# AY-Liu/Image-Editing-Framework

Measured on AMD Instinct MI355X. Metric: denoising steps/sec (SD1.5 512x512 P2P edit step, UNet batch 4), higher is better.
Workload: dtype f16x3; 1 GPU; sd15 UNet (859.5M params) P2P AttentionRefine edit step, 2 prompts x CFG = batch 4, 64x64 latents (512x512 px), 50-step DDIM, guidance 7.5, cross 0.8 / self 0.4, per-step null-text unconditional embeddings (P2P_NTI, edit_real.py); one independent edit per GPU; precision mode f16x3: fp32 storage; every contraction on split operands: hi + lo fp16 halves of each fp32 element, Ah Bh + Al Bh + Ah Bl =

## Files before the change

image-editing-framework_amd/csrc/split_x3.hip:

```cpp
#include "ief_common.h"
#include "ief_params.h"

#include "x3_common.h"

__global__ __launch_bounds__(256) void x3_split_weights_kernel(const float* __restrict__ w, half_t* __restrict__ planes, long long n4,
                                                               float s) {
    for (long long i = (long long)blockIdx.x * 256 + threadIdx.x; i < n4; i += (long long)gridDim.x * 256) {
        half4 h, l;
        split4(((const f32x4*)w)[i], s, h, l);
        ((half4*)planes)[i] = h;
        ((half4*)planes)[n4 + i] = l;
    }
}
extern "C" int ief_x3_split_weights(const float* w, void* planes, long long n, float scale, void* stream) {
    if (!w || !planes) return IEF_EINVAL;
    if (n <= 0 || (n & 3) || !(scale > 0.f)) return IEF_ESHAPE;
    long long grid = (n / 4 + 255) / 256;
    if (grid > 16384) grid = 16384;
    hipLaunchKernelGGL(x3_split_weights_kernel, dim3((unsigned)grid), dim3(256), 0, (hipStream_t)stream, w, (half_t*)planes, n / 4, scale);
    IEF_LAUNCH_CHECK();
    return IEF_OK;
}

template <int WM, int WN, int TM, int TN, int KIND, bool TRANSB, bool BPRE>
__global__ __launch_bounds__(64 * WM * WN, (2 * 2 * 16 * (WM * TM + WN * TN) * YLD * 2 > 80 * 1024) ? (WM * WN) / 4 : (WM * WN) / 2)
void igemm_x3_kernel(const IefGemmF32Params p) {
    constexpr bool CONV = KIND >= X3_CONV;
    constexpr bool HASFAST = KIND == X3_LIN || KIND == X3_CONV;
    constexpr int NTH = 64 * WM * WN;
    constexpr int BM = 16 * WM * TM, BN = 16 * WN * TN;
    constexpr int ROWS = BM + BN;
    constexpr int NA = (BM * 8 + NTH - 1) / NTH;
    constexpr int NBC = BPRE ? 2 * BN * 4 : BN * 8;
    constexpr int NB = (NBC + NTH - 1) / NTH;
    constexpr bool A_EXACT = (BM * 8) % NTH == 0, B_EXACT = NBC % NTH == 0;
    static_assert(!(BPRE && TRANSB), "pre-split planes are [N][K]");
    constexpr unsigned OOB = 0xFFFFFFF0u;
    constexpr unsigned OOBF = 0x80000000u;
    __shared__ __attribute__((aligned(16))) half_t smem_y[2 * 2 * ROWS * YLD];
    const int tid = threadIdx.x, lane = tid & 63, wid = tid >> 6;
    const int wm = wid / WN, wn = wid - wm * WN;
    const int lr = lane & 15, lg = lane >> 4;
    const int ntn = (p.N + BN - 1) / BN;
    const int ntiles = ((p.M + BM - 1) / BM) * ntn;
    const int bid = xcd_remap(blockIdx.x, ntiles);
    const int ntm = (p.M + BM - 1) / BM;
    const int grp = bid / (X3_GROUP_M * ntn), within = bid - grp * (X3_GROUP_M * ntn);
    const int gsz = min(X3_GROUP_M, ntm - grp * X3_GROUP_M);
    const int tn = within / gsz, tm = grp * X3_GROUP_M + (within - tn * gsz);
    const int m0 = tm * BM, n0 = tn * BN;
    const float* A = p.A;
    const float* W = p.W;
    float* Out = p.Out;
    if (p.heads > 0) {
        const int b = blockIdx.z / p.heads, h = blockIdx.z - b * p.heads;
        const int ba = p.a_src ? p.a_src[b] : b, bw = p.w_src ? p.w_src[b] : b;
        A += (long long)ba * p.sAb + (long long)h * p.sAh;
        W += (long long)bw * p.sWb + (long long)h * p.sWh;
        Out += (long long)b * p.sOb + (long long)h * p.sOh;
    }
    const int M = p.M, N = p.N, K = p.K;
    const float sa = p.sa, sb = p.sb;
    const int kc4 = (tid & 7) * 4;
    const int rq = tid >> 3;
    const int r0 = (rq & ~3) | ((rq & 1) << 1) | ((rq >> 1) & 1);
    constexpr int RSTEP = NTH / 8;
    RowCoordY rc[NA];
    unsigned pixo1[NA], pixo2[NA], tmask[NA];
    if (CONV) {
#pragma unroll
        for (int i = 0; i < NA; ++i) {
            const int m = m0 + r0 + RSTEP * i;
            rc[i].ok = m < M && (A_EXACT || r0 + RSTEP * i < BM);
            const int mm = rc[i].ok ? m : 0;
            const int hw = p.Ho * p.Wo;
            rc[i].b = mm / hw;
            const int rem = mm - rc[i].b * hw;
            rc[i].oy = rem / p.Wo;
            rc[i].ox = rem - rc[i].oy * p.Wo;
            if (KIND == X3_CONV) {
                const int pl = p.pad_hi_only ? 0 : 1;
                const unsigned pix = (unsigned)((rc[i].b * p.H + rc[i].oy * p.stride) * p.Wd + rc[i].ox * p.stride);
                pixo1[i] = pix * (unsigned)p.C1 * 4u; pixo2[i] = pix * (unsigned)p.C2 * 4u;
                unsigned mk = 0;
#pragma unroll
                for (int t = 0; t < 9; ++t) {
                    const int iy = rc[i].oy * p.stride + t / 3 - pl, ix = rc[i].ox * p.stride + t % 3 - pl;
                    mk |= (rc[i].ok && (unsigned)iy < (unsigned)p.H && (unsigned)ix < (unsigned)p.Wd) ? (1u << t) : 0u;
                }
                tmask[i] = mk;
            }
        }
    }
    const int Ct = p.C1 + p.C2, K9 = 9 * Ct;
    const int pad_lo = p.pad_hi_only ? 0 : 1;
    const int Hs = p.ups ? (p.H >> 1) : p.H, Ws = p.ups ? (p.Wd >> 1) : p.Wd;

    const int nk_all = (K + YBK - 1) / YBK;
    int kt0 = 0, nk = nk_all;
    if (p.splits > 1) {
        const int per = (nk_all + p.splits - 1) / p.splits;
        kt0 = blockIdx.y * per;
        nk = min(per, nk_all - kt0);
        if (nk < 0) nk = 0;
    }
    const int kend = min(K, (kt0 + nk) * YBK);

    const rsrc_t rA = make_rsrc(A, p.bytesA), rW = make_rsrc(BPRE ? (const void*)p.Wp : (const void*)W, p.bytesW);
    const rsrc_t rA2 = make_rsrc(p.A2, p.bytesA2), rE1 = make_rsrc(p.E1, p.bytesE1), rE2 = make_rsrc(p.E2, p.bytesE2);
    unsigned aoff[NA], boff[NB];
    bool aval[NA], bval[NB];
    int bq8[NB];
    int bldsoff[NB];
#pragma unroll
    for (int i = 0; i < NA; ++i) {
        const int ml = r0 + RSTEP * i, m = m0 + ml;
        aval[i] = (m < M) & (A_EXACT || ml < BM);
        aoff[i] = (unsigned)((m * p.lda + kc4) * 4);
    }
#pragma unroll
    for (int i = 0; i < NB; ++i) {
        bq8[i] = 0;
        if (BPRE) {
            const int c = tid + NTH * i;
            const int plane = c >= BN * 4 ? 1 : 0, cc = c - plane * BN * 4;
            const int rr = cc >> 2, q = cc & 3;
            const int nl = (rr & ~3) | ((rr & 1) << 1) | ((rr >> 1) & 1), n = n0 + nl;
            bval[i] = (c < NBC) & (n < N);
            bq8[i] = q * 8;
            boff[i] = (unsigned)(((long long)plane * N * K + (long long)n * K + q * 8) * 2);
            bldsoff[i] = plane * BN * YLD + nl * YLD + q * 8;
        } else if (!TRANSB) {
            const int nl = r0 + RSTEP * i, n = n0 + nl;
            bval[i] = (n < N) & (B_EXACT || nl < BN);
            boff[i] = (unsigned)((n * p.ldw + kc4) * 4);
            bldsoff[i] = nl * YLD + kc4;
        } else {
            const int c = tid + NTH * i;
            const int nl = (c >> 5) * 4, n = n0 + nl;
            bval[i] = (n < N) & (B_EXACT || nl < BN);
            boff[i] = (unsigned)(((c & 31) * p.ldw + n) * 4);
            bldsoff[i] = nl * YLD + (c & 31);
        }
    }

    auto load_tile = [&](int k0, f32x4 (&ra)[NA], f32x4 (&rb)[NB]) {
        const int kk = k0 + kc4;
        if (KIND == X3_CONV || KIND == X3_CONV_UPS) {
            int tap = 9, ch = k0 - K9;
            if (k0 < K9) { tap = k0 / Ct; ch = k0 - tap * Ct; }
            rsrc_t rs = rA;
            int cs = p.C1, chs = ch, ky = 0, kx = 0;
            const bool tapm = tap < 9;
            bool second = false;
            if (tapm) {
                ky = (tap * 11) >> 5; kx = tap - 3 * ky;
                if (ch >= p.C1) { rs = rA2; cs = p.C2; chs = ch - p.C1; second = true; }
            } else if (ch < p.CE1) { rs = rE1; cs = p.CE1; }
            else { rs = rE2; cs = p.CE2; chs = ch - p.CE1; }
            const int kin = k0 < kend ? 1 : 0;
            if (KIND == X3_CONV) {
                const int uni = tapm ? (((ky - pad_lo) * p.Wd + (kx - pad_lo)) * cs + chs) * 4 : chs * 4;
                const unsigned bit = tapm ? (1u << tap) : 0u;
                const unsigned cs4 = (unsigned)cs * 4u;
#pragma unroll
                for (int i = 0; i < NA; ++i) {
                    const unsigned base = tapm ? (second ? pixo2[i] : pixo1[i]) : (unsigned)(m0 + r0 + RSTEP * i) * cs4;
                    const bool ok = tapm ? (tmask[i] & bit) != 0 : rc[i].ok != 0;
                    ra[i] = bload(rs, (ok & (kin != 0)) ? base + (unsigned)uni + (unsigned)(kc4 * 4) : OOB);
                }
            } else {
                const int dy = tapm ? ky - pad_lo : 0, dx = tapm ? kx - pad_lo : 0;
                const unsigned Hc = tapm ? p.H : p.Ho, Wc = tapm ? p.Wd : p.Wo;
                const int sh = tapm ? 1 : 0;
                const int hs = tapm ? Hs : p.Ho, ws = tapm ? Ws : p.Wo;
                const int cb = chs + kc4;
#pragma unroll
                for (int i = 0; i < NA; ++i) {
                    const int iy = rc[i].oy + dy, ix = rc[i].ox + dx;
                    const int ok = rc[i].ok & kin & ((unsigned)iy < Hc ? 1 : 0) & ((unsigned)ix < Wc ? 1 : 0);
                    const unsigned off = (unsigned)((((rc[i].b * hs + (iy >> sh)) * ws + (ix >> sh)) * cs + cb) * 4);
                    ra[i] = bload(rs, ok ? off : OOB);
                }
            }
        } else if (KIND == X3_CONV_SLOW) {
            const float* src = nullptr;
            int cs = 0, chs = 0, ky = 0, kx = 0, mode = 0;
            if (kk < K9 && kk < kend) {
                const int tap = kk / Ct, ch = kk - tap * Ct;
                ky = tap / 3; kx = tap - 3 * ky;
                if (ch < p.C1) { src = p.A; cs = p.C1; chs = ch; } else { src = p.A2; cs = p.C2; chs = ch - p.C1; }
                mode = 1;
            } else if (kk < kend) {
                const int ch2 = kk - K9;
                if (ch2 < p.CE1) { src = p.E1; cs = p.CE1; chs = ch2; } else { src = p.E2; cs = p.CE2; chs = ch2 - p.CE1; }
                mode = 2;
            }
#pragma unroll
            for (int i = 0; i < NA; ++i) {
                f32x4 v = {0.f, 0.f, 0.f, 0.f};
                if (rc[i].ok && mode == 1) {
                    int iy = rc[i].oy * p.stride + ky - pad_lo, ix = rc[i].ox * p.stride + kx - pad_lo;
                    if ((unsigned)iy < (unsigned)p.H && (unsigned)ix < (unsigned)p.Wd) {
                        if (p.ups) { iy >>= 1; ix >>= 1; }
                        v = *(const f32x4*)(src + (((long long)rc[i].b * Hs + iy) * Ws + ix) * cs + chs);
                    }
                } else if (rc[i].ok && mode == 2) {
                    v = *(const f32x4*)(src + (((long long)rc[i].b * p.Ho + rc[i].oy) * p.Wo + rc[i].ox) * cs + chs);
                }
                ra[i] = v;
            }
        } else if (KIND == X3_LIN) {
#pragma unroll
            for (int i = 0; i < NA; ++i) ra[i] = bload(rA, (aval[i] & (kk < kend)) ? aoff[i] + (unsigned)(k0 * 4) : OOB);
        } else {
#pragma unroll
            for (int i = 0; i < NA; ++i) {
                const int m = m0 + r0 + RSTEP * i;
                f32x4 v = {0.f, 0.f, 0.f, 0.f};
                if (m < M && kk < kend && (A_EXACT || r0 + RSTEP * i < BM)) {
                    const float* ap = A + (long long)m * p.lda + kk;
#pragma unroll
                    for (int j = 0; j < 4; ++j) if (kk + j < K) v[j] = ap[j];
                }
                ra[i] = v;
            }
        }
        if (BPRE) {
#pragma unroll
            for (int i = 0; i < NB; ++i) rb[i] = bload(rW, (bval[i] & (k0 + bq8[i] < kend)) ? boff[i] + (unsigned)(k0 * 2) : OOB);
        } else if (!TRANSB) {
#pragma unroll
            for (int i = 0; i < NB; ++i) rb[i] = bload(rW, (bval[i] & (kk < kend)) ? boff[i] + (unsigned)(k0 * 4) : OOB);
        } else {
#pragma unroll
            for (int i = 0; i < NB; ++i) {
                const int kr = k0 + ((tid + NTH * i) & 31);
                rb[i] = bload(rW, (bval[i] & (kr < kend)) ? boff[i] + (unsigned)(k0 * p.ldw * 4) : OOB);
            }
        }
    };

    unsigned afast[NA], bfast[NB];
    rsrc_t f_rs = rA;
    int f_tap = 0, f_ch = 0, f_left = 0, f_uni = 0;
#pragma unroll
    for (int i = 0; i < NA; ++i) afast[i] = aval[i] ? aoff[i] : OOBF;
#pragma unroll
    for (int i = 0; i < NB; ++i) bfast[i] = bval[i] ? boff[i] : OOBF;
    auto seg_setup = [&]() {
        int cs, chs, src_c;
        const bool tapm = f_tap < 9;
        bool second = false;
        if (tapm) {
            if (f_ch >= p.C1) { f_rs = rA2; cs = p.C2; chs = f_ch - p.C1; second = true; src_c = p.C2; }
            else { f_rs = rA; cs = p.C1; chs = f_ch; src_c = p.C1; }
        } else if (f_ch < p.CE1) { f_rs = rE1; cs = p.CE1; chs = f_ch; src_c = p.CE1; }
        else { f_rs = rE2; cs = p.CE2; chs = f_ch - p.CE1; src_c = p.CE2; }
        f_left = (src_c - chs) / YBK;
        f_uni = chs * 4;
        const int ky = (f_tap * 11) >> 5, kx = f_tap - 3 * ky;
        const int tapoff = tapm ? ((ky - pad_lo) * p.Wd + (kx - pad_lo)) * cs * 4 : 0;
        const unsigned bit = tapm ? (1u << f_tap) : 0u;
#pragma unroll
        for (int i = 0; i < NA; ++i) {
            const unsigned base = tapm ? (second ? pixo2[i] : pixo1[i]) + (unsigned)tapoff
                                       : (unsigned)(m0 + r0 + RSTEP * i) * (unsigned)cs * 4u;
            const bool ok = tapm ? (tmask[i] & bit) != 0 : rc[i].ok != 0;
            afast[i] = ok ? base + (unsigned)(kc4 * 4) : OOBF;
        }
    };
    auto load_fast = [&](int k0, f32x4 (&ra)[NA], f32x4 (&rb)[NB]) {
        if (KIND == X3_CONV) {
#pragma unroll
            for (int i = 0; i < NA; ++i) ra[i] = bload(f_rs, afast[i] + (unsigned)f_uni);
            f_uni += YBK * 4;
            f_ch += YBK;
            if (--f_left == 0) {
                if (f_tap < 9 && f_ch >= Ct) { f_ch = 0; ++f_tap; }
                seg_setup();
            }
        } else {
#pragma unroll
            for (int i = 0; i < NA; ++i) ra[i] = bload(rA, afast[i] + (unsigned)(k0 * 4));
        }
        const unsigned kb = BPRE ? (unsigned)(k0 * 2) : TRANSB ? (unsigned)(k0 * p.ldw * 4) : (unsigned)(k0 * 4);
#pragma unroll
        for (int i = 0; i < NB; ++i) rb[i] = bload(rW, bfast[i] + kb);
    };

    auto store_chunk = [&](int buf, int idx, const f32x4 (&ra)[NA], const f32x4 (&rb)[NB]) {
        half_t* ah = smem_y + buf * (2 * ROWS * YLD);
        half_t* al = ah + BM * YLD;
        half_t* bh = al + BM * YLD;
        half_t* bl = bh + BN * YLD;
        if (idx < NA) {
            const int i = idx;
            if (!A_EXACT && r0 + RSTEP * i >= BM) return;
            half4 h, l;
            split4(ra[i], sa, h, l);
            const int off = (r0 + RSTEP * i) * YLD + kc4;
            *(half4*)(ah + off) = h;
            *(half4*)(al + off) = l;
        } else if (BPRE) {
            const int i = idx - NA;
            if (!B_EXACT && tid + NTH * i >= NBC) return;
            *(f32x4*)(bh + bldsoff[i]) = rb[i];
        } else if (!TRANSB) {
            const int i = idx - NA;
            if (!B_EXACT && r0 + RSTEP * i >= BN) return;
            half4 h, l;
            split4(rb[i], sb, h, l);
            *(half4*)(bh + bldsoff[i]) = h;
            *(half4*)(bl + bldsoff[i]) = l;
        } else {
            const int i = idx - NA;
            if (!B_EXACT && ((tid + NTH * i) >> 5) * 4 >= BN) return;
            half4 h, l;
            split4(rb[i], sb, h, l);
#pragma unroll
            for (int j = 0; j < 4; ++j) {
                bh[bldsoff[i] + j * YLD] = h[j];
                bl[bldsoff[i] + j * YLD] = l[j];
            }
        }
    };
    auto store_tile = [&](int buf, const f32x4 (&ra)[NA], const f32x4 (&rb)[NB]) {
#pragma unroll
        for (int c = 0; c < NA + NB; ++c) store_chunk(buf, c, ra, rb);
    };

    f32x4 acc[TN][TM];
#pragma unroll
    for (int b = 0; b < TN; ++b)
#pragma unroll
        for (int a = 0; a < TM; ++a) acc[b][a] = f32x4{0.f, 0.f, 0.f, 0.f};

    auto mma_tile = [&](int buf, const f32x4 (&ra)[NA], const f32x4 (&rb)[NB]) {
        const half_t* ah = smem_y + buf * (2 * ROWS * YLD) + (wm * TM * 16 + lr) * YLD + 8 * lg;
        const half_t* al = ah + BM * YLD;
        const half_t* bh = smem_y + buf * (2 * ROWS * YLD) + 2 * BM * YLD + (wn * TN * 16 + lr) * YLD + 8 * lg;
        const half_t* bl = bh + BN * YLD;
        half8_t fah[TM], fal[TM];
#pragma unroll
        for (int a = 0; a < TM; ++a) {
            fah[a] = *(const half8_t*)(ah + a * 16 * YLD);
            fal[a] = *(const half8_t*)(al + a * 16 * YLD);
        }
#pragma unroll
        for (int b = 0; b < TN; ++b) {
            const half8_t fbh = *(const half8_t*)(bh + b * 16 * YLD);
            const half8_t fbl = *(const half8_t*)(bl + b * 16 * YLD);
#pragma unroll
            for (int a = 0; a < TM; ++a) {
                acc[b][a] = __builtin_amdgcn_mfma_f32_16x16x32_f16(fbl, fah[a], acc[b][a], 0, 0, 0);
                acc[b][a] = __builtin_amdgcn_mfma_f32_16x16x32_f16(fbh, fal[a], acc[b][a], 0, 0, 0);
                acc[b][a] = __builtin_amdgcn_mfma_f32_16x16x32_f16(fbh, fah[a], acc[b][a], 0, 0, 0);
            }
        }
        store_tile(buf ^ 1, ra, rb);
    };

    f32x4 ra0[NA], rb0[NB], ra1[NA], rb1[NB];
    load_tile(kt0 * YBK, ra0, rb0);
    load_tile((kt0 + 1) * YBK, ra1, rb1);
    store_tile(0, ra0, rb0);
    __syncthreads();
    int kt = 0;
    if (HASFAST && p.fast_ok) {
        const int nfast = kend / YBK - kt0;
        if (KIND == X3_CONV && nfast > 3) {
            const int k0 = (kt0 + 2) * YBK;
            if (k0 < K9) { f_tap = k0 / Ct; f_ch = k0 - f_tap * Ct; } else { f_tap = 9; f_ch = k0 - K9; }
            seg_setup();
        }
        for (; kt + 3 < nfast; kt += 2) {
            load_fast((kt0 + kt + 2) * YBK, ra0, rb0);
            mma_tile(0, ra1, rb1);
            __syncthreads();
            load_fast((kt0 + kt + 3) * YBK, ra1, rb1);
            mma_tile(1, ra0, rb0);
            __syncthreads();
        }
    }
    for (; kt < nk; kt += 2) {
        load_tile((kt0 + kt + 2) * YBK, ra0, rb0);
        mma_tile(0, ra1, rb1);
        __syncthreads();
        load_tile((kt0 + kt + 3) * YBK, ra1, rb1);
        mma_tile(1, ra0, rb0);
        __syncthreads();
    }
    const float inv = 1.0f / (sa * sb);
    const bool vec = p.vec_out != 0;
    if (p.splits > 1) {
        float* slab = p.ws + (long long)blockIdx.y * M * N;
#pragma unroll
        for (int a = 0; a < TM; ++a) {
            const int m = m0 + (wm * TM + a) * 16 + lr;
            if (m >= M) continue;
#pragma unroll
            for (int b = 0; b < TN; ++b) {
                const int n = n0 + (wn * TN + b) * 16 + 4 * lg;
                if (n >= N) continue;
                const f32x4 v = acc[b][a] * inv;
                if ((N & 3) == 0) *(f32x4*)(slab + (long long)m * N + n) = v;
                else {
#pragma unroll
                    for (int j = 0; j < 4; ++j) if (n + j < N) slab[(long long)m * N + n + j] = v[j];
                }
            }
        }
        return;
    }
    if (p.geglu) {
#pragma unroll
        for (int a = 0; a < TM; ++a) {
            const int m = m0 + (wm * TM + a) * 16 + lr;
#pragma unroll
            for (int b = 0; b < TN; ++b) {
                const int n = n0 + (wn * TN + b) * 16 + 4 * lg;
                f32x4 v = acc[b][a] * inv;
                if (p.bias && n < N) v += *(const f32x4*)(p.bias + n);
                f32x4 g;
#pragma unroll
                for (int j = 0; j < 4; ++j) g[j] = __shfl_xor(v[j], 32);
                if (lg < 2 && m < M && n < N) {
                    f32x4 o;
#pragma unroll
                    for (int j = 0; j < 4; ++j) o[j] = v[j] * gelu_f(g[j]) * p.out_scale;
                    *(f32x4*)(Out + (long long)m * p.ldo + (n0 + (wn * TN + b) * 16) / 2 + 4 * lg) = o;
                }
            }
        }
        return;
    }
    const float* R = p.residual;
#pragma unroll
    for (int a = 0; a < TM; ++a) {
        const int m = m0 + (wm * TM + a) * 16 + lr;
        if (m >= M) continue;
        const float* rv = p.rowvec ? p.rowvec + (long long)(m / p.rows_per_batch) * N : nullptr;
#pragma unroll
        for (int b = 0; b < TN; ++b) {
            const int n = n0 + (wn * TN + b) * 16 + 4 * lg;
            if (n >= N) continue;
            f32x4 v = acc[b][a] * inv;
            if (vec) {
                if (p.bias) v += *(const f32x4*)(p.bias + n);
                if (rv) v += *(const f32x4*)(rv + n);
                if (R) v += *(const f32x4*)(R + (long long)m * p.ldr + n);
                *(f32x4*)(Out + (long long)m * p.ldo + n) = v * p.out_scale;
            } else {
#pragma unroll
                for (int j = 0; j < 4; ++j) {
                    if (n + j >= N) break;
                    float s = v[j];
                    if (p.bias) s += p.bias[n + j];
                    if (rv) s += rv[n + j];
                    if (R) s += R[(long long)m * p.ldr + n + j];
                    Out[(long long)m * p.ldo + n + j] = s * p.out_scale;
                }
            }
        }
    }
}

static int g_x3_wide = 1, g_flash_ks2 = 1;
extern "C" void ief_gemm_x3_set_variant(int v) { g_x3_wide = v & 1; g_flash_ks2 = (v & 2) ? 0 : 1; }
static bool x3_wide_ok(int conv, int N, int K) { return g_x3_wide && N % 160 == 0 && (conv || N <= 1280 || K >= 1280); }
extern "C" int ief_gemm_x3_bn_k(int conv, int N, int K) { return x3_wide_ok(conv, N, K) ? 160 : (N % 80 == 0) ? 80 : 64; }
extern "C" int ief_gemm_x3_bn(int N) { return (N % 80 == 0) ? 80 : 64; }
extern "C" int ief_gemm_x3_bm(int M, int N) {
    (void)M; (void)N;
    return 128;
}

template <int WM, int WN, int TM, int TN, int KIND, bool TRANSB, bool BPRE>
static int launch_igemm_x3(const IefGemmF32Params& p, hipStream_t st) {
    constexpr int BM = 16 * WM * TM, BN = 16 * WN * TN;
    const int tiles = ((p.M + BM - 1) / BM) * ((p.N + BN - 1) / BN);
    const int z = p.heads > 0 ? p.batch * p.heads : 1;
    const int splits = p.splits > 1 ? p.splits : 1;
    hipLaunchKernelGGL((igemm_x3_kernel<WM, WN, TM, TN, KIND, TRANSB, BPRE>), dim3(tiles, splits, z), dim3(64 * WM * WN), 0, st, p);
    IEF_LAUNCH_CHECK();
    return IEF_OK;
}

int ief_gemm_x3_dispatch(const IefGemmF32Params& pin, hipStream_t st) {
    IefGemmF32Params p = pin;
    const bool al = ((p.N & 3) == 0) && ((p.ldo & 3) == 0) && (((uintptr_t)p.Out & 15) == 0) &&
                    (!p.bias || ((uintptr_t)p.bias & 15) == 0) && (!p.rowvec || ((uintptr_t)p.rowvec & 15) == 0) &&
                    (!p.residual || (((uintptr_t)p.residual & 15) == 0 && (p.ldr & 3) == 0)) &&
                    (p.heads == 0 || (((p.sOb | p.sOh) & 3) == 0));
    p.vec_out = al ? 1 : 0;
    if (p.geglu && (p.conv || p.transb || p.heads > 0 || p.splits > 1 || (p.N & 15) || p.residual || p.rowvec || !al ||
                    (((uintptr_t)p.Out | (uintptr_t)(p.bias ? p.bias : p.Out)) & 15) || (p.ldo & 3)))
        return IEF_EINVAL;
    const bool bpre = p.Wp != nullptr;
    if (bpre && (p.transb || p.heads > 0 || (p.K & 7) || ((uintptr_t)p.Wp & 15) || (!p.conv && p.ldw != p.K))) return IEF_EINVAL;
    const unsigned long long lim = 0xFFFFFFF0ull;
    unsigned long long bA, bW, bA2 = 0, bE1 = 0, bE2 = 0;
    if (p.conv) {
        const unsigned long long px = (unsigned long long)p.batch_images * (p.ups ? (p.H >> 1) * (p.Wd >> 1) : p.H * p.Wd);
        bA = px * p.C1 * 4; bA2 = px * p.C2 * 4;
        bE1 = (unsigned long long)p.M * p.CE1 * 4; bE2 = (unsigned long long)p.M * p.CE2 * 4;
        p.al32 = ((p.C1 | p.C2 | p.CE1 | p.CE2) & 31) == 0 ? 1 : 0;
    } else {
        bA = ((unsigned long long)(p.M - 1) * p.lda + p.K) * 4;
        p.al32 = 0;
    }
    bW = bpre ? 4ull * p.N * p.K
              : p.transb ? ((unsigned long long)(p.K - 1) * p.ldw + p.N) * 4 : ((unsigned long long)(p.N - 1) * p.ldw + p.K) * 4;
    if (bA >= lim || bW >= lim || bA2 >= lim || bE1 >= lim || bE2 >= lim) return IEF_ESHAPE;
    p.bytesA = (unsigned)bA; p.bytesW = (unsigned)bW; p.bytesA2 = (unsigned)bA2; p.bytesE1 = (unsigned)bE1; p.bytesE2 = (unsigned)bE2;
    const unsigned long long half = 0x40000000ull;
    const unsigned long long kspan = p.transb ? 4ull * p.K * p.ldw : 4ull * p.K;
    p.fast_ok = (bA < half && bW < half && bA2 < half && bE1 < half && bE2 < half && kspan < half) ? 1 : 0;
    if (x3_wide_ok(p.conv, p.N, p.K) && bpre && !p.a_scalar && (!p.conv || (p.al32 && !p.ups)))
        return p.conv ? launch_igemm_x3<4, 2, 2, 5, X3_CONV, false, true>(p, st) : launch_igemm_x3<4, 2, 2, 5, X3_LIN, false, true>(p, st);
    const bool n80 = p.N % 80 == 0;
#define X3_GO(KIND_, TRANSB_, BPRE_) (n80 ? launch_igemm_x3<4, 1, 2, 5, KIND_, TRANSB_, BPRE_>(p, st) \
                                          : launch_igemm_x3<2, 2, 4, 2, KIND_, TRANSB_, BPRE_>(p, st))
    if (p.conv) {
        if (!p.al32) return bpre ? X3_GO(X3_CONV_SLOW, false, true) : X3_GO(X3_CONV_SLOW, false, false);
        if (p.ups) return bpre ? X3_GO(X3_CONV_UPS, false, true) : X3_GO(X3_CONV_UPS, false, false);
        return bpre ? X3_GO(X3_CONV, false, true) : X3_GO(X3_CONV, false, false);
    }
    if (p.transb) return p.a_scalar ? X3_GO(X3_LIN_SLOW, true, false) : X3_GO(X3_LIN, true, false);
    if (p.a_scalar) return bpre ? X3_GO(X3_LIN_SLOW, false, true) : X3_GO(X3_LIN_SLOW, false, false);
    return bpre ? X3_GO(X3_LIN, false, true) : X3_GO(X3_LIN, false, false);
#undef X3_GO
}

template <int D, int KS>
__global__ __launch_bounds__(256, (D > 80) ? 1 : 2) void attn_flash_x3_kernel(const IefAttnF32Params p) {
    constexpr int DG = (D + 15) / 16;
    constexpr int DT = (D + 31) / 32;
    constexpr int KLD = DG * 16 + 8;
    constexpr int KT = 32 * KS;
    constexpr int VRS = D <= 32 ? 32 : (D <= 96 ? 96 : 160);
    static_assert(VRS >= 32 * DT, "V row covers the padded head dim");
    constexpr float SQ = 1.f, SK = 1.f, SV = 1.f, SP = 16384.f;
    __shared__ __attribute__((aligned(16))) half_t smem_f[2 * KT * KLD + 2 * KT * VRS];
    half_t* Kh = smem_f;
    half_t* Kl = Kh + KT * KLD;
    half_t* Vh = Kl + KT * KLD;
    half_t* Vl = Vh + KT * VRS;
    const int tid = threadIdx.x, lane = tid & 63, wid = tid >> 6;
    const int li = lane & 31, lh = lane >> 5;
    const int nqb = gridDim.x;
    const int lid = xcd_remap(blockIdx.x + nqb * blockIdx.y, nqb * gridDim.y);
    const int bh = lid / nqb, qb = lid - bh * nqb, b = bh / p.heads, h = bh - b * p.heads;
    const int bq = p.q_src ? p.q_src[b] : b, bk = p.k_src ? p.k_src[b] : b, bv = p.v_src ? p.v_src[b] : b;
    const float* Q = p.Q + (long long)bq * p.sQb + (long long)h * D;
    const float* Kp = p.K + (long long)bk * p.sKb + (long long)h * D;
    const float* Vp = p.V + (long long)bv * p.sVb + (long long)h * D;
    float* O = p.Out ? p.Out + (long long)b * p.sOb + (long long)h * D : nullptr;
    half_t* OP = p.OutP ? p.OutP + (long long)b * p.sOPb + (long long)h * D : nullptr;
    const int q0 = qb * 128 + wid * 32;
    const int qi = q0 + li;
    for (int c = tid; c < (int)(sizeof(smem_f) / 16); c += 256) ((f32x4*)smem_f)[c] = f32x4{0.f, 0.f, 0.f, 0.f};
    half8_t qh[DG], ql[DG];
#pragma unroll
    for (int g = 0; g < DG; ++g) {
#pragma unroll
        for (int c2 = 0; c2 < 2; ++c2) {
            const int d0 = g * 16 + 8 * lh + 4 * c2;
            f32x4 v = {0.f, 0.f, 0.f, 0.f};
            if (qi < p.N && d0 < D) v = *(const f32x4*)(Q + (long long)qi * p.ldq + d0);
            half4 hh, ll;
            split4(v, SQ, hh, ll);
#pragma unroll
            for (int j = 0; j < 4; ++j) { qh[g][4 * c2 + j] = hh[j]; ql[g][4 * c2 + j] = ll[j]; }
        }
    }
    f32x16 o[DT];
#pragma unroll
    for (int t = 0; t < DT; ++t)
#pragma unroll
        for (int r = 0; r < 16; ++r) o[t][r] = 0.f;
    float m_run = -INFINITY, l_run = 0.f;
    const float sc2 = p.scale * 1.44269504088896341f / (SQ * SK);
    constexpr int KCH = KT * (D / 4);
    constexpr int NLD = (KCH + 255) / 256;
    const rsrc_t rK = make_rsrc(Kp, (unsigned)(((long long)(p.L - 1) * p.ldk + D) * 4));
    const rsrc_t rV = make_rsrc(Vp, (unsigned)(((long long)(p.L - 1) * p.ldv + D) * 4));
    f32x4 rk[NLD], rv[NLD];
    auto load_kv = [&](int k0) {
#pragma unroll
        for (int i = 0; i < NLD; ++i) {
            const int c = tid + 256 * i;
            const int row = c / (D / 4), ch = c - row * (D / 4);
            const bool ok = (c < KCH) & (k0 + row < p.L);
            rk[i] = bload(rK, ok ? (unsigned)(((k0 + row) * p.ldk + ch * 4) * 4) : 0xFFFFFFF0u);
            rv[i] = bload(rV, ok ? (unsigned)(((k0 + row) * p.ldv + ch * 4) * 4) : 0xFFFFFFF0u);
        }
    };
    auto store_kv = [&]() {
#pragma unroll
        for (int i = 0; i < NLD; ++i) {
            const int c = tid + 256 * i;
            if (c < KCH) {
                const int row = c / (D / 4), ch = c - row * (D / 4);
                half4 hh, ll;
                split4(rk[i], SK, hh, ll);
                *(half4*)(Kh + row * KLD + ch * 4) = hh;
                *(half4*)(Kl + row * KLD + ch * 4) = ll;
                split4(rv[i], SV, hh, ll);
                *(half4*)(Vh + row * VRS + ch * 4) = hh;
                *(half4*)(Vl + row * VRS + ch * 4) = ll;
            }
        }
    };
    const int L16 = lane & 15;
    const int v_lane = (4 * lh + (L16 >> 2)) * VRS + 16 * ((lane >> 4) & 1) + 4 * (L16 & 3);
    const int nt = (p.L + KT - 1) / KT;
    load_kv(0);
    for (int t = 0; t < nt; ++t) {
        __syncthreads();
        store_kv();
        __syncthreads();
        load_kv((t + 1) * KT);
        f32x16 sacc[KS];
#pragma unroll
        for (int u = 0; u < KS; ++u) {
#pragma unroll
            for (int r = 0; r < 16; ++r) sacc[u][r] = 0.f;
#pragma unroll
            for (int g = 0; g < DG; ++g) {
                const half8_t kh = *(const half8_t*)(Kh + (u * 32 + li) * KLD + g * 16 + 8 * lh);
                const half8_t kl = *(const half8_t*)(Kl + (u * 32 + li) * KLD + g * 16 + 8 * lh);
                sacc[u] = __builtin_amdgcn_mfma_f32_32x32x16_f16(kl, qh[g], sacc[u], 0, 0, 0);
                sacc[u] = __builtin_amdgcn_mfma_f32_32x32x16_f16(kh, ql[g], sacc[u], 0, 0, 0);
                sacc[u] = __builtin_amdgcn_mfma_f32_32x32x16_f16(kh, qh[g], sacc[u], 0, 0, 0);
            }
        }
#pragma unroll
        for (int u = 0; u < KS; ++u) {
            if (t * KT + (u + 1) * 32 > p.L) {
#pragma unroll
                for (int r = 0; r < 16; ++r) {
                    const int key = t * KT + u * 32 + (r & 3) + 8 * (r >> 2) + 4 * lh;
                    if (key >= p.L) sacc[u][r] = -INFINITY;
                }
            }
        }
        float mxa = -INFINITY, mxb = -INFINITY;
#pragma unroll
        for (int r = 0; r < 8; ++r) {
            if (KS == 2) {
                mxa = __builtin_fmaxf(__builtin_fmaxf(mxa, sacc[0][r]), sacc[KS - 1][r]);
                mxb = __builtin_fmaxf(__builtin_fmaxf(mxb, sacc[0][8 + r]), sacc[KS - 1][8 + r]);
            } else {
                mxa = __builtin_fmaxf(mxa, sacc[0][r]);
                mxb = __builtin_fmaxf(mxb, sacc[0][8 + r]);
            }
        }
        float mx = fmaxf(mxa, mxb) * sc2;
        mx = fmaxf(mx, __shfl_xor(mx, 32));
        const float m_new = fmaxf(m_run, mx);
        const float alpha = __builtin_amdgcn_exp2f(m_run - m_new);
        float ls = 0.f;
#pragma unroll
        for (int u = 0; u < KS; ++u)
#pragma unroll
            for (int r = 0; r < 16; ++r) { sacc[u][r] = __builtin_amdgcn_exp2f(__builtin_fmaf(sacc[u][r], sc2, -m_new)); ls += sacc[u][r]; }
        l_run = l_run * alpha + ls;
        if (__builtin_amdgcn_ballot_w64(m_new != m_run) != 0) {
#pragma unroll
            for (int tt = 0; tt < DT; ++tt)
#pragma unroll
                for (int r = 0; r < 16; ++r) o[tt][r] *= alpha;
        }
        m_run = m_new;
#pragma unroll
        for (int u = 0; u < KS; ++u) {
#pragma unroll
            for (int s = 0; s < 2; ++s) {
                half8_t ph, pl;
#pragma unroll
                for (int c2 = 0; c2 < 2; ++c2) {
                    const f32x4 v = {sacc[u][8 * s + 4 * c2], sacc[u][8 * s + 4 * c2 + 1], sacc[u][8 * s + 4 * c2 + 2], sacc[u][8 * s + 4 * c2 + 3]};
                    half4 hh, ll;
                    split4(v, SP, hh, ll);
#pragma unroll
                    for (int j = 0; j < 4; ++j) { ph[4 * c2 + j] = hh[j]; pl[4 * c2 + j] = ll[j]; }
                }
#pragma unroll
                for (int tt = 0; tt < DT; ++tt) {
                    const int vo = v_lane + (u * 32 + 16 * s) * VRS + 32 * tt;
                    const half4 a0 = x3_lds_tr_read(Vh + vo), a1 = x3_lds_tr_read(Vh + vo + 8 * VRS);
                    const half4 b0 = x3_lds_tr_read(Vl + vo), b1 = x3_lds_tr_read(Vl + vo + 8 * VRS);
                    half8_t vh, vl;
#pragma unroll
                    for (int j = 0; j < 4; ++j) { vh[j] = a0[j]; vh[4 + j] = a1[j]; vl[j] = b0[j]; vl[4 + j] = b1[j]; }
                    o[tt] = __builtin_amdgcn_mfma_f32_32x32x16_f16(vl, ph, o[tt], 0, 0, 0);
                    o[tt] = __builtin_amdgcn_mfma_f32_32x32x16_f16(vh, pl, o[tt], 0, 0, 0);
                    o[tt] = __builtin_amdgcn_mfma_f32_32x32x16_f16(vh, ph, o[tt], 0, 0, 0);
                }
            }
        }
    }
    const float l_tot = l_run + __shfl_xor(l_run, 32);
    const float inv = 1.0f / (l_tot * SV * SP);
    if (p.lse && qi < p.N && lh == 0) p.lse[((long long)b * p.heads + h) * p.N + qi] = m_run + __log2f(l_tot);
    if (qi < p.N) {
#pragma unroll
        for (int tt = 0; tt < DT; ++tt)
#pragma unroll
            for (int g = 0; g < 4; ++g) {
                const int d = tt * 32 + 8 * g + 4 * lh;
                if (d < D) {
                    const f32x4 v = {o[tt][4 * g] * inv, o[tt][4 * g + 1] * inv, o[tt][4 * g + 2] * inv, o[tt][4 * g + 3] * inv};
                    if (O) *(f32x4*)(O + (long long)qi * p.ldo + d) = v;
                    if (OP) {
                        half4 hh, ll;
                        split4(v, 1.0f, hh, ll);
                        half_t* op = OP + (long long)qi * p.ldp + d;
                        *(half4*)op = hh;
                        *(half4*)(op + p.planeO) = ll;
                    }
                }
            }
    }
}


#ifndef X3P_FLASH_BATCH_READS
#define X3P_FLASH_BATCH_READS 1
#endif
template <int D, int KS, int NWV>
__global__ __launch_bounds__(64 * NWV, D <= 40 ? 4 : 2) void attn_flash_x3p_kernel(const IefAttnF32Params p) {
    constexpr int DG = (D + 15) / 16, DT = (D + 31) / 32;
    constexpr int KT = 32 * KS;
    constexpr int CPR = D / 8;
    constexpr int PL = KT * D;
    constexpr int NP = PL * 2 / 1024;
    static_assert((PL * 2) % 1024 == 0, "a plane of a tile is a whole number of LDS-DMA pieces");
    constexpr bool SWZ = D == 64;
    constexpr float LOGSP = 10.f, THR = 5.f;
    constexpr bool BATCH_READS = X3P_FLASH_BATCH_READS != 0;
    __shared__ __attribute__((aligned(1024))) half_t smem_p[2 * 4 * PL];
    const int tid = threadIdx.x, lane = tid & 63;
    const int wid = __builtin_amdgcn_readfirstlane(tid >> 6);
    const int li = lane & 31, lh = lane >> 5;
    const int nqb = gridDim.x;
    const int lid = xcd_remap(blockIdx.x + nqb * blockIdx.y, nqb * gridDim.y);
    const int bh = lid / nqb, qb = lid - bh * nqb, b = bh / p.heads, h = bh - b * p.heads;
    const int bq = p.q_src ? p.q_src[b] : b, bk = p.k_src ? p.k_src[b] : b, bv = p.v_src ? p.v_src[b] : b;
    const half_t* Qh = p.Qp + (long long)bq * p.sQb + (long long)h * D;
    const char* srcs[4];
#pragma unroll
    for (int pl = 0; pl < 4; ++pl)
        srcs[pl] = (const char*)(pl < 2 ? p.Kp + (long long)bk * p.sKb + (pl & 1) * p.planeK
                                        : p.Vp + (long long)bv * p.sVb + (pl & 1) * p.planeV) + (long long)h * D * 2;
    const char* zp = (const char*)p.zeros;
    float* O = p.Out ? p.Out + (long long)b * p.sOb + (long long)h * D : nullptr;
    half_t* OP = p.OutP ? p.OutP + (long long)b * p.sOPb + (long long)h * D : nullptr;
    const int q0 = qb * (32 * NWV) + wid * 32;
    const int qi = q0 + li;
    half8_t qh[DG], ql[DG];
#pragma unroll
    for (int g = 0; g < DG; ++g) {
        const int d0 = g * 16 + 8 * lh;
        if (qi < p.N && d0 < D) {
            qh[g] = *(const half8_t*)(Qh + (long long)qi * p.ldq + d0);
            ql[g] = *(const half8_t*)(Qh + p.planeQ + (long long)qi * p.ldq + d0);
        } else {
#pragma unroll
            for (int j = 0; j < 8; ++j) { qh[g][j] = 0; ql[g][j] = 0; }
        }
    }
    constexpr int NPW = (4 * NP + NWV - 1) / NWV;
    int s_row[NPW];
    unsigned s_off[NPW];
#pragma unroll
    for (int i = 0; i < NPW; ++i) {
        const int q = wid + NWV * i, j = q % NP;
        const int c = 64 * j + lane;
        s_row[i] = c / CPR;
        const int ch = c - s_row[i] * CPR;
        s_off[i] = (unsigned)((SWZ ? (ch ^ (s_row[i] & 7)) : ch) * 16);
    }
    auto issue = [&](int t, int buf) {
#pragma unroll
        for (int i = 0; i < NPW; ++i) {
            const int q = wid + NWV * i;
            if (q < 4 * NP) {
                const int pl = q / NP, j = q - pl * NP;
                const int row = t * KT + s_row[i];
                const int ldr = pl < 2 ? p.ldk : p.ldv;
                const char* g = row < p.L ? srcs[pl] + (long long)row * ldr * 2 + s_off[i] : zp;
                x3_glds16(g, smem_p + buf * (4 * PL) + pl * PL + j * 512);
            }
        }
    };
    int koff[DG];
#pragma unroll
    for (int g = 0; g < DG; ++g) {
        const int chunk = (g * 16 + 8 * lh < D) ? 2 * g + lh : 0;
        koff[g] = li * D + (SWZ ? ((chunk ^ (li & 7)) << 3) : (chunk << 3));
    }
    const int L16 = lane & 15;
    const int vrow = 4 * lh + (L16 >> 2);
    int voff[DT];
#pragma unroll
    for (int tt = 0; tt < DT; ++tt) {
        int col = 32 * tt + 16 * ((lane >> 4) & 1) + 4 * (L16 & 3);
        if (col >= D) col = 0;
        voff[tt] = col;
    }
    f32x16 o[DT];
#pragma unroll
    for (int t = 0; t < DT; ++t)
#pragma unroll
        for (int r = 0; r < 16; ++r) o[t][r] = 0.f;
    float m_run = -INFINITY, l_run = 0.f;
    const float sc2 = p.scale * 1.44269504088896341f;
    const int nt = (p.L + KT - 1) / KT;
    issue(0, 0);
    for (int t = 0; t < nt; ++t) {
        asm volatile("s_waitcnt vmcnt(0)" ::: "memory");
        __syncthreads();
        if (t + 1 < nt) issue(t + 1, (t + 1) & 1);
        const half_t* Kh = smem_p + (t & 1) * (4 * PL);
        const half_t* Kl = Kh + PL;
        const half_t* Vh = Kl + PL;
        const half_t* Vl = Vh + PL;
        __builtin_amdgcn_s_setprio(1);
        f32x16 sacc[KS];
#pragma unroll
        for (int u = 0; u < KS; ++u) {
#pragma unroll
            for (int r = 0; r < 16; ++r) sacc[u][r] = 0.f;
            half8_t kh[DG], kl[DG];
#pragma unroll
            for (int g = 0; g < DG; ++g) {
                kh[g] = *(const half8_t*)(Kh + u * 32 * D + koff[g]);
                kl[g] = *(const half8_t*)(Kl + u * 32 * D + koff[g]);
            }
            if constexpr (BATCH_READS) __builtin_amdgcn_sched_barrier(0);
#pragma unroll
            for (int g = 0; g < DG; ++g) {
                sacc[u] = __builtin_amdgcn_mfma_f32_32x32x16_f16(kl[g], qh[g], sacc[u], 0, 0, 0);
                sacc[u] = __builtin_amdgcn_mfma_f32_32x32x16_f16(kh[g], ql[g], sacc[u], 0, 0, 0);
                sacc[u] = __builtin_amdgcn_mfma_f32_32x32x16_f16(kh[g], qh[g], sacc[u], 0, 0, 0);
            }
            if constexpr (BATCH_READS) __builtin_amdgcn_sched_barrier(0);
        }
        __builtin_amdgcn_s_setprio(0);
#pragma unroll
        for (int u = 0; u < KS; ++u) {
            if (t * KT + (u + 1) * 32 > p.L) {
#pragma unroll
                for (int r = 0; r < 16; ++r) {
                    const int key = t * KT + u * 32 + (r & 3) + 8 * (r >> 2) + 4 * lh;
                    if (key >= p.L) sacc[u][r] = -INFINITY;
                }
            }
        }
        float mxa = -INFINITY, mxb = -INFINITY;
#pragma unroll
        for (int r = 0; r < 8; ++r) {
            if (KS == 2) {
                mxa = __builtin_fmaxf(__builtin_fmaxf(mxa, sacc[0][r]), sacc[KS - 1][r]);
                mxb = __builtin_fmaxf(__builtin_fmaxf(mxb, sacc[0][8 + r]), sacc[KS - 1][8 + r]);
            } else {
                mxa = __builtin_fmaxf(mxa, sacc[0][r]);
                mxb = __builtin_fmaxf(mxb, sacc[0][8 + r]);
            }
        }
        float mx = fmaxf(mxa, mxb) * sc2;
        if (__builtin_amdgcn_ballot_w64(mx > m_run + THR) != 0) {
            mx = fmaxf(mx, __shfl_xor(mx, 32));
            const float m_new = fmaxf(m_run, mx);
            const float alpha = __builtin_amdgcn_exp2f(m_run - m_new);
#pragma unroll
            for (int tt = 0; tt < DT; ++tt)
#pragma unroll
                for (int r = 0; r < 16; ++r) o[tt][r] *= alpha;
            l_run *= alpha;
            m_run = m_new;
        }
        const float mb = LOGSP - m_run;
        float ls = 0.f;
#pragma unroll
        for (int u = 0; u < KS; ++u)
#pragma unroll
            for (int r = 0; r < 16; ++r) { sacc[u][r] = __builtin_amdgcn_exp2f(__builtin_fmaf(sacc[u][r], sc2, mb)); ls += sacc[u][r]; }
        l_run += ls;
        __builtin_amdgcn_s_setprio(1);
#pragma unroll
        for (int u = 0; u < KS; ++u) {
#pragma unroll
            for (int s2 = 0; s2 < 2; ++s2) {
                half8_t ph, pl;
#pragma unroll
                for (int c2 = 0; c2 < 2; ++c2) {
                    const f32x4 v = {sacc[u][8 * s2 + 4 * c2], sacc[u][8 * s2 + 4 * c2 + 1], sacc[u][8 * s2 + 4 * c2 + 2], sacc[u][8 * s2 + 4 * c2 + 3]};
                    half4 hh, ll;
                    split4(v, 1.0f, hh, ll);
#pragma unroll
                    for (int j = 0; j < 4; ++j) { ph[4 * c2 + j] = hh[j]; pl[4 * c2 + j] = ll[j]; }
                }
                half8_t vh[DT], vl[DT];
#pragma unroll
                for (int tt = 0; tt < DT; ++tt) {
                    const int r0 = u * 32 + 16 * s2 + vrow;
                    const int c = voff[tt];
                    const int o0 = r0 * D + (SWZ ? ((((c >> 3) ^ (r0 & 7)) << 3) | (c & 7)) : c);
                    const int o1 = (r0 + 8) * D + (SWZ ? ((((c >> 3) ^ ((r0 + 8) & 7)) << 3) | (c & 7)) : c);
                    const half4 a0 = x3_lds_tr_read(Vh + o0), a1 = x3_lds_tr_read(Vh + o1);
                    const half4 b0 = x3_lds_tr_read(Vl + o0), b1 = x3_lds_tr_read(Vl + o1);
#pragma unroll
                    for (int j = 0; j < 4; ++j) { vh[tt][j] = a0[j]; vh[tt][4 + j] = a1[j]; vl[tt][j] = b0[j]; vl[tt][4 + j] = b1[j]; }
                }
                if constexpr (BATCH_READS) __builtin_amdgcn_sched_barrier(0);
#pragma unroll
                for (int tt = 0; tt < DT; ++tt) {
                    o[tt] = __builtin_amdgcn_mfma_f32_32x32x16_f16(vl[tt], ph, o[tt], 0, 0, 0);
                    o[tt] = __builtin_amdgcn_mfma_f32_32x32x16_f16(vh[tt], pl, o[tt], 0, 0, 0);
                    o[tt] = __builtin_amdgcn_mfma_f32_32x32x16_f16(vh[tt], ph, o[tt], 0, 0, 0);
                }
                if constexpr (BATCH_READS) __builtin_amdgcn_sched_barrier(0);
            }
        }
        __builtin_amdgcn_s_setprio(0);
    }
    const float l_tot = l_run + __shfl_xor(l_run, 32);
    const float inv = 1.0f / l_tot;
    if (qi < p.N) {
#pragma unroll
        for (int tt = 0; tt < DT; ++tt)
#pragma unroll
            for (int g = 0; g < 4; ++g) {
                const int d = tt * 32 + 8 * g + 4 * lh;
                if (d < D) {
                    const f32x4 v = {o[tt][4 * g] * inv, o[tt][4 * g + 1] * inv, o[tt][4 * g + 2] * inv, o[tt][4 * g + 3] * inv};
                    if (O) *(f32x4*)(O + (long long)qi * p.ldo + d) = v;
                    if (OP) {
                        half4 hh, ll;
                        split4(v, 1.0f, hh, ll);
                        half_t* op = OP + (long long)qi * p.ldp + d;
                        *(half4*)op = hh;
                        *(half4*)(op + p.planeO) = ll;
                    }
                }
            }
    }
}

int ief_attn_flash_x3_dispatch(const IefAttnF32Params& p, hipStream_t st) {
    if (p.Out && ((p.ldo & 3) || (p.sOb & 3) || ((uintptr_t)p.Out & 15))) return IEF_EALIGN;
    if (p.OutP && ((p.ldp & 3) || (p.sOPb & 3) || (p.planeO & 3) || ((uintptr_t)p.OutP & 7))) return IEF_EALIGN;
    const unsigned long long lim = 0xFFFFFFF0ull;
    if (((unsigned long long)(p.L - 1) * p.ldk + p.d) * 4 >= lim || ((unsigned long long)(p.L - 1) * p.ldv + p.d) * 4 >= lim) return IEF_ESHAPE;
    dim3 grid((p.N + 127) / 128, p.B * p.heads);
    if (p.Qp) {
        const dim3 grid8((p.N + 255) / 256, p.B * p.heads);
        if (!p.Kp || !p.Vp || !p.zeros) return IEF_EINVAL;
        if ((p.ldq & 7) || (p.ldk & 7) || (p.ldv & 7) || (p.sQb & 7) || (p.sKb & 7) || (p.sVb & 7) || (p.planeQ & 7) || (p.planeK & 7) ||
            (p.planeV & 7) || (((uintptr_t)p.Qp | (uintptr_t)p.Kp | (uintptr_t)p.Vp) & 15)) return IEF_EALIGN;
        switch (p.d) {
            case 40: hipLaunchKernelGGL((attn_flash_x3p_kernel<40, 2, 8>), grid8, dim3(512), 0, st, p); break;
            case 64: hipLaunchKernelGGL((attn_flash_x3p_kernel<64, 1, 4>), grid, dim3(256), 0, st, p); break;
            case 80: hipLaunchKernelGGL((attn_flash_x3p_kernel<80, 1, 4>), grid, dim3(256), 0, st, p); break;
            default: return IEF_ESHAPE;
        }
        IEF_LAUNCH_CHECK();
        return IEF_OK;
    }
    const bool ks2 = g_flash_ks2 && p.L >= 128;
#define FLASH_GO(D_) do { if (ks2) hipLaunchKernelGGL((attn_flash_x3_kernel<D_, 2>), grid, dim3(256), 0, st, p); \
                          else hipLaunchKernelGGL((attn_flash_x3_kernel<D_, 1>), grid, dim3(256), 0, st, p); } while (0)
    switch (p.d) {
        case 32: FLASH_GO(32); break;
        case 40: FLASH_GO(40); break;
        case 64: FLASH_GO(64); break;
        case 80: FLASH_GO(80); break;
        case 160: FLASH_GO(160); break;
        default: return IEF_ESHAPE;
    }
    IEF_LAUNCH_CHECK();
    return IEF_OK;
}
```

image-editing-framework_amd/csrc/x3_common.h:

```cpp
#pragma once
#include "ief_common.h"

#define YBK 32
#ifndef X3_GROUP_M
#define X3_GROUP_M 8
#endif
#define YLD 48

typedef __attribute__((ext_vector_type(8))) _Float16 half8_t;
typedef __attribute__((ext_vector_type(2))) float f32x2;

struct RowCoordY { int b, oy, ox, ok; };

typedef __amdgpu_buffer_rsrc_t rsrc_t;
__device__ __forceinline__ rsrc_t make_rsrc(const void* p, unsigned bytes) {
    return __builtin_amdgcn_make_buffer_rsrc(const_cast<void*>(p), 0, (int)bytes, 0x00020000);
}
__device__ __forceinline__ f32x4 bload(rsrc_t r, unsigned off) {
    return __builtin_bit_cast(f32x4, __builtin_amdgcn_raw_buffer_load_b128(r, (int)off, 0, 0));
}

__device__ __forceinline__ void split4(const f32x4 v, const float s, half4& hi, half4& lo) {
    const f32x4 x = v * s;
    const half2_t h0 = __builtin_convertvector(f32x2{x[0], x[1]}, half2_t);
    const half2_t h1 = __builtin_convertvector(f32x2{x[2], x[3]}, half2_t);
    float r0, r1, r2, r3;
    asm("v_fma_mix_f32 %0, %1, 1.0, -%2 op_sel:[0,0,0] op_sel_hi:[0,0,1]" : "=v"(r0) : "v"(x[0]), "v"(h0));
    asm("v_fma_mix_f32 %0, %1, 1.0, -%2 op_sel:[0,0,1] op_sel_hi:[0,0,1]" : "=v"(r1) : "v"(x[1]), "v"(h0));
    asm("v_fma_mix_f32 %0, %1, 1.0, -%2 op_sel:[0,0,0] op_sel_hi:[0,0,1]" : "=v"(r2) : "v"(x[2]), "v"(h1));
    asm("v_fma_mix_f32 %0, %1, 1.0, -%2 op_sel:[0,0,1] op_sel_hi:[0,0,1]" : "=v"(r3) : "v"(x[3]), "v"(h1));
    const half2_t l0 = __builtin_convertvector(f32x2{r0, r1}, half2_t);
    const half2_t l1 = __builtin_convertvector(f32x2{r2, r3}, half2_t);
    hi = half4{h0[0], h0[1], h1[0], h1[1]};
    lo = half4{l0[0], l0[1], l1[0], l1[1]};
}

typedef __fp16 x3_fp16x4_t __attribute__((__vector_size__(4 * sizeof(__fp16))));
typedef __attribute__((address_space(3))) x3_fp16x4_t x3_lds_fp16x4_t;
__device__ __forceinline__ half4 x3_lds_tr_read(const half_t* p) {
    const x3_fp16x4_t v = __builtin_amdgcn_ds_read_tr16_b64_v4f16((x3_lds_fp16x4_t*)p);
    return __builtin_bit_cast(half4, v);
}

__device__ __forceinline__ void x3_glds16(const char* g, half_t* lds_wave_base) {
    __builtin_amdgcn_global_load_lds((const __attribute__((address_space(1))) void*)g, (__attribute__((address_space(3))) void*)lds_wave_base, 16, 0, 0);
}

enum { X3_LIN = 0, X3_LIN_SLOW = 1, X3_CONV = 2, X3_CONV_UPS = 3, X3_CONV_SLOW = 4 };
```

Baseline: 73.78 steps/s.

## Fold softmax scale, max bias and row sum into MFMA padding lanes for D%16 heads

For head dimensions not a multiple of 16 (e.g. SD1.5's 40), the flash attention kernel now uses the otherwise-zero padded K/Q lanes to carry a bias term. The query is prescaled by the softmax scale and the running max offset is injected through the padded column, so the per-element FMA before exp2 disappears. A ones column appended to V makes the PV MFMA also accumulate the row sum, which removes the separate l_run reduction. In exchange the V tiles in LDS are wider, bias updates are quantised to 1/256, and numerical precision shifts slightly.

```diff
diff --git a/image-editing-framework_amd/csrc/split_x3.hip b/image-editing-framework_amd/csrc/split_x3.hip
--- a/image-editing-framework_amd/csrc/split_x3.hip
+++ b/image-editing-framework_amd/csrc/split_x3.hip
@@ -734,14 +734,20 @@
 __global__ __launch_bounds__(64 * NWV, D <= 40 ? 4 : 2) void attn_flash_x3p_kernel(const IefAttnF32Params p) {
     constexpr int DG = (D + 15) / 16, DT = (D + 31) / 32;
     constexpr int KT = 32 * KS;
+    constexpr bool FOLD = D % 16 != 0;
     constexpr int CPR = D / 8;
+    constexpr int VR = FOLD ? D + 8 : D;
+    constexpr int VCPR = VR / 8;
     constexpr int PL = KT * D;
-    constexpr int NP = PL * 2 / 1024;
-    static_assert((PL * 2) % 1024 == 0, "a plane of a tile is a whole number of LDS-DMA pieces");
+    constexpr int PLV = KT * VR;
+    constexpr int NPK = PL * 2 / 1024, NPV = PLV * 2 / 1024;
+    constexpr int NPT = 2 * NPK + 2 * NPV;
+    constexpr int BUF = 2 * PL + 2 * PLV;
+    static_assert((PL * 2) % 1024 == 0 && (PLV * 2) % 1024 == 0, "a plane of a tile is a whole number of LDS-DMA pieces");
     constexpr bool SWZ = D == 64;
     constexpr float LOGSP = 10.f, THR = 5.f;
     constexpr bool BATCH_READS = X3P_FLASH_BATCH_READS != 0;
-    __shared__ __attribute__((aligned(1024))) half_t smem_p[2 * 4 * PL];
+    __shared__ __attribute__((aligned(1024))) half_t smem_p[2 * BUF];
     const int tid = threadIdx.x, lane = tid & 63;
     const int wid = __builtin_amdgcn_readfirstlane(tid >> 6);
     const int li = lane & 31, lh = lane >> 5;
@@ -772,27 +778,51 @@
             for (int j = 0; j < 8; ++j) { qh[g][j] = 0; ql[g][j] = 0; }
         }
     }
-    constexpr int NPW = (4 * NP + NWV - 1) / NWV;
+    if constexpr (FOLD) {
+        const float sc2 = p.scale * 1.44269504088896341f;
+#pragma unroll
+        for (int g = 0; g < DG; ++g)
+#pragma unroll
+            for (int j = 0; j < 8; ++j) {
+                const float x = ((float)qh[g][j] + (float)ql[g][j]) * sc2;
+                qh[g][j] = (half_t)x;
+                ql[g][j] = (half_t)(x - (float)qh[g][j]);
+            }
+        for (int r = tid; r < 2 * 2 * KT; r += 64 * NWV) {
+            const int bp = r / KT;
+            half8_t c = {};
+            if ((bp & 1) == 0) c[0] = (half_t)1.0f;
+            *(half8_t*)(smem_p + (bp >> 1) * BUF + 2 * PL + (bp & 1) * PLV + (r - bp * KT) * VR + D) = c;
+        }
+    }
+    constexpr int NPW = (NPT + NWV - 1) / NWV;
     int s_row[NPW];
     unsigned s_off[NPW];
+    bool s_pad[NPW];
 #pragma unroll
     for (int i = 0; i < NPW; ++i) {
-        const int q = wid + NWV * i, j = q % NP;
+        const int q = wid + NWV * i;
+        const bool kp = !FOLD || q < 2 * NPK;
+        const int j = kp ? q % NPK : (q - 2 * NPK) % NPV, cpr = kp ? CPR : VCPR;
         const int c = 64 * j + lane;
-        s_row[i] = c / CPR;
-        const int ch = c - s_row[i] * CPR;
+        s_row[i] = c / cpr;
+        const int ch = c - s_row[i] * cpr;
+        s_pad[i] = ch >= CPR;
         s_off[i] = (unsigned)((SWZ ? (ch ^ (s_row[i] & 7)) : ch) * 16);
     }
     auto issue = [&](int t, int buf) {
 #pragma unroll
         for (int i = 0; i < NPW; ++i) {
             const int q = wid + NWV * i;
-            if (q < 4 * NP) {
-                const int pl = q / NP, j = q - pl * NP;
+            if (q < NPT) {
+                const bool kp = !FOLD || q < 2 * NPK;
+                const int pl = kp ? q / NPK : 2 + (q - 2 * NPK) / NPV;
+                const int j = kp ? q - pl * NPK : q - 2 * NPK - (pl - 2) * NPV;
                 const int row = t * KT + s_row[i];
                 const int ldr = pl < 2 ? p.ldk : p.ldv;
                 const char* g = row < p.L ? srcs[pl] + (long long)row * ldr * 2 + s_off[i] : zp;
-                x3_glds16(g, smem_p + buf * (4 * PL) + pl * PL + j * 512);
+                half_t* dst = smem_p + buf * BUF + (kp ? pl * PL : 2 * PL + (pl - 2) * PLV) + j * 512;
+                if (!FOLD || !s_pad[i]) x3_glds16(g, dst);
             }
         }
     };
@@ -808,7 +838,7 @@
 #pragma unroll
     for (int tt = 0; tt < DT; ++tt) {
         int col = 32 * tt + 16 * ((lane >> 4) & 1) + 4 * (L16 & 3);
-        if (col >= D) col = 0;
+        if (col >= VR) col = 0;
         voff[tt] = col;
     }
     f32x16 o[DT];
@@ -816,18 +846,24 @@
     for (int t = 0; t < DT; ++t)
 #pragma unroll
         for (int r = 0; r < 16; ++r) o[t][r] = 0.f;
-    float m_run = -INFINITY, l_run = 0.f;
+    float m_run = FOLD ? 0.f : -INFINITY, l_run = 0.f;
     const float sc2 = p.scale * 1.44269504088896341f;
+    auto set_bias = [&]() {
+        const float bb = 0.5f * (LOGSP - m_run);
+        const half_t bh = (half_t)bb, bl = (half_t)(bb - (float)bh);
+        if (lh) { qh[DG - 1][1] = bh; ql[DG - 1][1] = bl; }
+    };
+    if constexpr (FOLD) set_bias();
     const int nt = (p.L + KT - 1) / KT;
     issue(0, 0);
     for (int t = 0; t < nt; ++t) {
         asm volatile("s_waitcnt vmcnt(0)" ::: "memory");
         __syncthreads();
         if (t + 1 < nt) issue(t + 1, (t + 1) & 1);
-        const half_t* Kh = smem_p + (t & 1) * (4 * PL);
+        const half_t* Kh = smem_p + (t & 1) * BUF;
         const half_t* Kl = Kh + PL;
         const half_t* Vh = Kl + PL;
-        const half_t* Vl = Vh + PL;
+        const half_t* Vl = Vh + PLV;
         __builtin_amdgcn_s_setprio(1);
         f32x16 sacc[KS];
 #pragma unroll
@@ -841,6 +877,13 @@
                 kl[g] = *(const half8_t*)(Kl + u * 32 * D + koff[g]);
             }
             if constexpr (BATCH_READS) __builtin_amdgcn_sched_barrier(0);
+            if constexpr (FOLD) {
+                x3_u32x4 wh = __builtin_bit_cast(x3_u32x4, kh[DG - 1]), wl = __builtin_bit_cast(x3_u32x4, kl[DG - 1]);
+                wh[0] = lh ? 0x40000000u : wh[0];
+                wl[0] = lh ? 0u : wl[0];
+                kh[DG - 1] = __builtin_bit_cast(half8_t, wh);
+                kl[DG - 1] = __builtin_bit_cast(half8_t, wl);
+            }
 #pragma unroll
             for (int g = 0; g < DG; ++g) {
                 sacc[u] = __builtin_amdgcn_mfma_f32_32x32x16_f16(kl[g], qh[g], sacc[u], 0, 0, 0);
@@ -871,25 +914,52 @@
                 mxb = __builtin_fmaxf(mxb, sacc[0][8 + r]);
             }
         }
-        float mx = fmaxf(mxa, mxb) * sc2;
-        if (__builtin_amdgcn_ballot_w64(mx > m_run + THR) != 0) {
-            mx = fmaxf(mx, __shfl_xor(mx, 32));
-            const float m_new = fmaxf(m_run, mx);
-            const float alpha = __builtin_amdgcn_exp2f(m_run - m_new);
-#pragma unroll
-            for (int tt = 0; tt < DT; ++tt)
-#pragma unroll
-                for (int r = 0; r < 16; ++r) o[tt][r] *= alpha;
-            l_run *= alpha;
-            m_run = m_new;
-        }
-        const float mb = LOGSP - m_run;
-        float ls = 0.f;
-#pragma unroll
-        for (int u = 0; u < KS; ++u)
-#pragma unroll
-            for (int r = 0; r < 16; ++r) { sacc[u][r] = __builtin_amdgcn_exp2f(__builtin_fmaf(sacc[u][r], sc2, mb)); ls += sacc[u][r]; }
-        l_run += ls;
+        if constexpr (FOLD) {
+            float mx = fmaxf(mxa, mxb);
+            if (__builtin_amdgcn_ballot_w64(mx > LOGSP + THR) != 0 || t == 0) {
+                mx = fmaxf(mx, __shfl_xor(mx, 32)) - LOGSP + m_run;
+                float m_new = t ? fmaxf(m_run, mx) : mx;
+                m_new = __builtin_ceilf(m_new * 256.f) * (1.f / 256.f);
+                if (t) {
+                    const float alpha = __builtin_amdgcn_exp2f(m_run - m_new);
+#pragma unroll
+                    for (int tt = 0; tt < DT; ++tt)
+#pragma unroll
+                        for (int r = 0; r < 16; ++r) o[tt][r] *= alpha;
+                }
+                const float sh = m_new - m_run;
+#pragma unroll
+                for (int u = 0; u < KS; ++u)
+#pragma unroll
+                    for (int r = 0; r < 16; ++r) sacc[u][r] -= sh;
+                m_run = m_new;
+                set_bias();
+            }
+#pragma unroll
+            for (int u = 0; u < KS; ++u)
+#pragma unroll
+                for (int r = 0; r < 16; ++r) sacc[u][r] = __builtin_amdgcn_exp2f(sacc[u][r]);
+        } else {
+            float mx = fmaxf(mxa, mxb) * sc2;
+            if (__builtin_amdgcn_ballot_w64(mx > m_run + THR) != 0) {
+                mx = fmaxf(mx, __shfl_xor(mx, 32));
+                const float m_new = fmaxf(m_run, mx);
+                const float alpha = __builtin_amdgcn_exp2f(m_run - m_new);
+#pragma unroll
+                for (int tt = 0; tt < DT; ++tt)
+#pragma unroll
+                    for (int r = 0; r < 16; ++r) o[tt][r] *= alpha;
+                l_run *= alpha;
+                m_run = m_new;
+            }
+            const float mb = LOGSP - m_run;
+            float ls = 0.f;
+#pragma unroll
+            for (int u = 0; u < KS; ++u)
+#pragma unroll
+                for (int r = 0; r < 16; ++r) { sacc[u][r] = __builtin_amdgcn_exp2f(__builtin_fmaf(sacc[u][r], sc2, mb)); ls += sacc[u][r]; }
+            l_run += ls;
+        }
         __builtin_amdgcn_s_setprio(1);
 #pragma unroll
         for (int u = 0; u < KS; ++u) {
@@ -909,8 +979,8 @@
                 for (int tt = 0; tt < DT; ++tt) {
                     const int r0 = u * 32 + 16 * s2 + vrow;
                     const int c = voff[tt];
-                    const int o0 = r0 * D + (SWZ ? ((((c >> 3) ^ (r0 & 7)) << 3) | (c & 7)) : c);
-                    const int o1 = (r0 + 8) * D + (SWZ ? ((((c >> 3) ^ ((r0 + 8) & 7)) << 3) | (c & 7)) : c);
+                    const int o0 = r0 * VR + (SWZ ? ((((c >> 3) ^ (r0 & 7)) << 3) | (c & 7)) : c);
+                    const int o1 = (r0 + 8) * VR + (SWZ ? ((((c >> 3) ^ ((r0 + 8) & 7)) << 3) | (c & 7)) : c);
                     const half4 a0 = x3_lds_tr_read(Vh + o0), a1 = x3_lds_tr_read(Vh + o1);
                     const half4 b0 = x3_lds_tr_read(Vl + o0), b1 = x3_lds_tr_read(Vl + o1);
 #pragma unroll
@@ -928,7 +998,14 @@
         }
         __builtin_amdgcn_s_setprio(0);
     }
-    const float l_tot = l_run + __shfl_xor(l_run, 32);
+    float l_tot;
+    if constexpr (FOLD) {
+        constexpr int RD = D % 32, REG = 4 * (RD / 8) + RD % 4, LHD = (RD % 8) / 4;
+        const float lr = o[D / 32][REG], lx = __shfl_xor(lr, 32);
+        l_tot = lh == LHD ? lr : lx;
+    } else {
+        l_tot = l_run + __shfl_xor(l_run, 32);
+    }
     const float inv = 1.0f / l_tot;
     if (qi < p.N) {
 #pragma unroll
diff --git a/image-editing-framework_amd/csrc/x3_common.h b/image-editing-framework_amd/csrc/x3_common.h
--- a/image-editing-framework_amd/csrc/x3_common.h
+++ b/image-editing-framework_amd/csrc/x3_common.h
@@ -9,6 +9,7 @@
 
 typedef __attribute__((ext_vector_type(8))) _Float16 half8_t;
 typedef __attribute__((ext_vector_type(2))) float f32x2;
+typedef __attribute__((ext_vector_type(4))) unsigned x3_u32x4;
 
 struct RowCoordY { int b, oy, ox, ok; };
 
```

Result: no change. 74.23 steps/s (median of 6 runs) (+0.6%).
